# LuChengTHU/dpm-solver

Hardware: NVIDIA H100
Metric: solver-update GElem/s (higher is better)
Workload: dtype bf16

## Files before the change

dpm_solver_b200/_lib.py:

```python
from __future__ import annotations

import ctypes as C
import os
from pathlib import Path

_PKG = Path(__file__).resolve().parent
LIB_PATH = _PKG / "lib" / "libdpmsolver_b200.so"

DPM_F32, DPM_BF16, DPM_F16 = 0, 1, 2
FORM_NONE, FORM_LIN1, FORM_LIN2, FORM_LIN3, FORM_DIFF2, FORM_MS3, FORM_SS3T = range(7)
PARAM_NOISE, PARAM_X_START, PARAM_V, PARAM_SCORE = range(4)

PARAM_BY_NAME = {"noise": PARAM_NOISE, "x_start": PARAM_X_START, "v": PARAM_V, "score": PARAM_SCORE}


class StepDesc(C.Structure):
    _fields_ = [
        ("x", C.c_void_p), ("xe", C.c_void_p), ("m0", C.c_void_p), ("m1", C.c_void_p),
        ("m2", C.c_void_p), ("m_out", C.c_void_p), ("out", C.c_void_p), ("out2", C.c_void_p),
        ("e_cond", C.c_void_p), ("e_uncond", C.c_void_p), ("thr", C.c_void_p),
        ("n", C.c_uint64), ("per_sample", C.c_uint64),
        ("state_dtype", C.c_int32), ("model_dtype", C.c_int32), ("form", C.c_int32),
        ("n_model", C.c_int32), ("param", C.c_int32), ("predict_x0", C.c_int32),
        ("c0_on_old", C.c_int32), ("raw_round", C.c_int32),
# ... 41 lines not shown
    "dpm_dynamic_threshold_workspace": (C.c_size_t, [_u64, _u64]),
    "dpm_dynamic_threshold": (C.c_int, [_vp, C.POINTER(StepDesc), _f, _f, _vp, C.c_size_t, _vp]),
    "dpm_adaptive_init": (C.c_int, [C.POINTER(AdaptiveCtl), _f, _f, _vp]),
    "dpm_adaptive_plan": (C.c_int, [C.POINTER(AdaptiveCtl), _vp]),
    "dpm_adaptive_decide": (C.c_int, [C.POINTER(AdaptiveCtl), _vp]),
    "dpm_select_copy": (C.c_int, [_vp, _vp, _vp, _u64, _vp]),
    "dpm_adaptive_error_workspace": (C.c_size_t, [_u64, _u64]),
    "dpm_adaptive_error": (C.c_int, [_vp, _vp, _vp, _vp, _f, _f, _u64, _u64, _i, _vp, C.c_size_t, _vp]),
    "dpm_cfg_rescale_workspace": (C.c_size_t, [_u64, _u64]),
    "dpm_cfg_rescale_ratio": (C.c_int, [_vp, _vp, _vp, _f, _u64, _u64, _i, _vp, C.c_size_t, _vp]),
    "dpm_step_rescaled": (C.c_int, [C.POINTER(StepDesc), _vp, _f, _f, _vp]),
    "dpm_step_guided": (C.c_int, [C.POINTER(StepDesc), _vp, _vp, _f, _f, _vp]),
    "dpm_cfg_rescale_ratio_guided": (C.c_int, [_vp, _vp, _vp, _vp, _u64, _u64, _i, _vp, C.c_size_t, _vp]),
    "dpm_step_multi": (C.c_int, [C.POINTER(StepDesc), C.POINTER(_vp), C.POINTER(_f), _i, C.POINTER(_vp), _vp]),
    "dpm_replicate": (C.c_int, [_vp, _vp, _u64, _i, _i, _vp]),
}

MAX_CONDITIONS = 4

_lib = None


class DpmLibraryError(RuntimeError):
    pass


def lib() -> C.CDLL:
    global _lib
    if _lib is not None:
        return _lib
# ... 22 lines not shown
```

dpm_solver_b200/build.py:

```python
from __future__ import annotations

import argparse
import hashlib
import os
import shutil
import subprocess
import sys
from concurrent.futures import ThreadPoolExecutor
from pathlib import Path

PKG = Path(__file__).resolve().parent
ROOT = PKG.parent
CSRC = PKG / "csrc"
INCLUDE = ROOT / "include"
OUT_DIR = PKG / "lib"
BUILD_DIR = PKG / "build"
LIB_NAME = "libdpmsolver_b200.so"

SOURCES = ["capi.cu", "step_direct.cu", "step_multi.cu", "step_tma.cu","quantile.cu", "adaptive.cu", "adaptive_ctl.cu", "philox.cu"]
FMAD_DEFAULT = {"philox.cu"}
ARCH = ["-gencode", "arch=compute_90a,code=sm_90a"]
NVCC_FLAGS = ["-O3", "-std=c++17", "-lineinfo", "-fmad=false", "-Xcompiler", "-fPIC",
              "-Xcompiler", "-fvisibility=hidden", "--expt-relaxed-constexpr"]


def _nvcc() -> str:
    for cand in (os.environ.get("NVCC"), shutil.which("nvcc"), "/usr/local/cuda/bin/nvcc"):
        if cand and Path(cand).exists():
            return cand
    raise RuntimeError("nvcc not found (set NVCC=/path/to/nvcc)")


def _stamp(extra: list[str]) -> str:
    h = hashlib.sha256()
# ... 62 lines not shown
```

dpm_solver_b200/csrc/capi.cu:

```cuda
#include <atomic>
#include <mutex>
#include <set>
#include <utility>
#include <cstdarg>
#include <cstdio>
#include <cstdlib>
#include <cstring>

#include "launch.cuh"

namespace dpm {

static thread_local char g_err[512] = "";
static std::atomic<uint64_t> g_launches{0};
static std::atomic<int> g_variant{2}, g_threads{0}, g_ctas{0};

void set_error(const char* fmt, ...) {
  va_list ap;
  va_start(ap, fmt);
  vsnprintf(g_err, sizeof(g_err), fmt, ap);
  va_end(ap);
}
void count_launch() { g_launches.fetch_add(1, std::memory_order_relaxed); }
bool pdl_enabled() {
// ... 260 lines not shown
  Tuning t{g_variant.load(), g_threads.load(), g_ctas.load()};
  bool body_done = false;
  if (mp.k.npk > 0 && aligned_all && mp.k.dev_coef == nullptr) {
    const int r = launch_step_multi(mp, t, stream);
    if (r < 0 || r > 1) return r;
    body_done = (r == 0);
  }
  if (!body_done) {
    rc = launch_step_multi_scalar(mp, stream);
  } else if (mp.k.n % kPacket) {
    rc = launch_step_multi_scalar(shifted_multi(mp, (uint64_t)mp.k.npk * kPacket), stream);
  }
  return finish(rc);
}

}

using namespace dpm;

extern "C" {

int dpm_version(void) { return DPM_B200_VERSION; }
const char* dpm_last_error(void) { return g_err; }
uint64_t dpm_launch_count(void) { return g_launches.load(); }

int dpm_set_tuning(int variant, int threads, int ctas_per_sm) {
  if (variant < 0 || variant > 2) { set_error("variant must be 0 (direct), 1 (TMA ring) or 2 (auto)"); return DPM_ERR_ARG; }
  if (threads != 0 && (threads < 32 || threads > 512 || threads % 32)) { set_error("threads must be a multiple of 32 in [32,512]"); return DPM_ERR_ARG; }
  if (ctas_per_sm < 0 || ctas_per_sm > 32) { set_error("ctas_per_sm must be in [0,32]"); return DPM_ERR_ARG; }
  g_variant = variant; g_threads = threads; g_ctas = ctas_per_sm;
// ... 135 lines not shown
  if (out == nullptr || x == nullptr || !valid_dtype(dtype)) { set_error("duplicate: NULL tensor or bad dtype"); return DPM_ERR_ARG; }
  cudaStream_t st = static_cast<cudaStream_t>(stream);
  const uint64_t bytes = n * (uint64_t)esize(dtype);
  int r = launch_duplicate(out, x, bytes, st);
  if (r == 1) {
    cudaError_t e = cudaMemcpyAsync(out, x, bytes, cudaMemcpyDeviceToDevice, st);
    if (e == cudaSuccess) e = cudaMemcpyAsync(static_cast<char*>(out) + bytes, x, bytes, cudaMemcpyDeviceToDevice, st);
    return e != cudaSuccess ? launch_error("duplicate", e) : DPM_OK;
  }
  return finish(r);
}

int dpm_step_multi(const dpm_step_desc* desc, const void* const* e_conds, const float* scales, int n_cond,
                   void* const* replicas, dpm_stream_t stream) {
  return step_multi_impl(desc, e_conds, scales, n_cond, replicas, static_cast<cudaStream_t>(stream));
}

int dpm_replicate(void* out, const void* x, uint64_t n, int copies, int dtype, dpm_stream_t stream) {
  if (copies < 1 || out == nullptr || x == nullptr || !valid_dtype(dtype)) {
    set_error("replicate: NULL tensor, bad dtype or copies < 1");
    return DPM_ERR_ARG;
  }
  if (n == 0) return DPM_OK;
  cudaStream_t st = static_cast<cudaStream_t>(stream);
  const uint64_t bytes = n * (uint64_t)esize(dtype);
  int r = launch_replicate(out, x, bytes, copies, st);
  if (r == 1) {
    cudaError_t e = cudaSuccess;
    for (int c = 0; c < copies && e == cudaSuccess; ++c)
      e = cudaMemcpyAsync(static_cast<char*>(out) + (uint64_t)c * bytes, x, bytes, cudaMemcpyDeviceToDevice, st);
// ... 75 lines not shown
```

dpm_solver_b200/csrc/common.cuh:

```cuda
#pragma once
#include <cuda_bf16.h>
#include <cuda_fp16.h>
#include <cuda_runtime.h>
#include <stdint.h>
#include <string.h>

#include "dpm_solver_b200.h"

namespace dpm {

constexpr int kPacket = 8;

struct KParams {
  const void* x;
  const void* xe;
  const void* m0;
  const void* m1;
  const void* m2;
  const void* ec;
  const void* eu;
  void* m_out;
  void* out;
  void* out2;
  const float* thr;
// ... 21 lines not shown
  const float* dev_coef;
  const float* ratio;
  float phi, psi;
  const float* gscale;
};

constexpr int kMaxCond = DPM_MAX_CONDITIONS;
struct MultiParams {
  KParams k;
  const void* ec[kMaxCond];
  void* rep[kMaxCond];
  float s[kMaxCond];
  int32_t n_cond;
};

template <typename T> struct Raw;
template <> struct Raw<float> { uint32_t r[8]; };
template <> struct Raw<__nv_bfloat16> { uint32_t r[4]; };
template <> struct Raw<__half> { uint32_t r[4]; };

template <typename T> struct Traits;
template <> struct Traits<float> { static constexpr int kBytes = 4; static constexpr int kCode = DPM_F32; };
template <> struct Traits<__nv_bfloat16> { static constexpr int kBytes = 2; static constexpr int kCode = DPM_BF16; };
template <> struct Traits<__half> { static constexpr int kBytes = 2; static constexpr int kCode = DPM_F16; };

__device__ __forceinline__ void ldg_pk(Raw<float>& v, const float* p) {
  asm volatile("ld.global.L1::no_allocate.v4.b32 {%0,%1,%2,%3}, [%8];\n\t"
               "ld.global.L1::no_allocate.v4.b32 {%4,%5,%6,%7}, [%8+16];"
               : "=r"(v.r[0]), "=r"(v.r[1]), "=r"(v.r[2]), "=r"(v.r[3]), "=r"(v.r[4]),
                 "=r"(v.r[5]), "=r"(v.r[6]), "=r"(v.r[7])
// ... 357 lines not shown
```

dpm_solver_b200/csrc/launch.cuh:

```cuda
#pragma once
#include <cuda_runtime.h>
#include <stdint.h>

#include <type_traits>

#include "common.cuh"

namespace dpm {

struct Tuning {
  int variant;
  int threads;
  int ctas_per_sm;
};

int sm_count();
int max_smem_optin();
void count_launch();
int ensure_max_smem(const void* kernel, bool nonportable_cluster = false);
void set_error(const char* fmt, ...);
int launch_error(const char* what, cudaError_t e);

template <typename TE_, typename TS_> struct PacketPair {
  using TE = TE_;
// ... 64 lines not shown
int launch_step_direct(const KParams& p, const Tuning& t, cudaStream_t stream);
int launch_step_scalar(const KParams& p, cudaStream_t stream);
int launch_step_tma(const KParams& p, const Tuning& t, cudaStream_t stream);
void philox_policy(uint64_t numel, uint32_t* grid, uint64_t* counter_offset);
int launch_noise_philox(void* out, const void* x, const void* xt, const float* mask, uint64_t mask_n, uint64_t n,
                        int t_count, const float* alpha, const float* sigma, uint64_t seed, uint64_t offset,
                        int x_dtype, int out_dtype, cudaStream_t stream);
int launch_adaptive_init(const dpm_adaptive_ctl* a, float t_T, float h_init, cudaStream_t stream);
int launch_adaptive_plan(const dpm_adaptive_ctl* a, cudaStream_t stream);
int launch_adaptive_decide(const dpm_adaptive_ctl* a, cudaStream_t stream);
int launch_select_copy(void* dst, const void* src, const float* state, uint64_t bytes, cudaStream_t stream);
int launch_duplicate(void* dst, const void* src, uint64_t bytes, cudaStream_t stream);
int launch_step_multi(const MultiParams& mp, const Tuning& t, cudaStream_t stream);
int launch_step_multi_scalar(const MultiParams& mp, cudaStream_t stream);
int launch_replicate(void* dst, const void* src, uint64_t bytes, int copies, cudaStream_t stream);
int launch_quantile(float* s_out, const KParams& p, uint64_t n_samples, float q, float max_val,
                    void* workspace, size_t workspace_bytes, cudaStream_t stream);
size_t quantile_workspace_bytes(uint64_t n_samples, uint64_t per_sample);
size_t adaptive_workspace_bytes(uint64_t n, uint64_t per_sample);
int launch_adaptive_error(float* out, const void* xh, const void* xl, const void* xp, float atol, float rtol,
                          uint64_t per_sample, uint64_t n, int dtype, void* ws, size_t ws_bytes, cudaStream_t stream);
size_t cfg_rescale_workspace_bytes(uint64_t n_samples, uint64_t per_sample);
int launch_cfg_rescale_ratio(float* ratio, const void* ec, const void* eu, float guidance, uint64_t per_sample,
                             uint64_t n, int dtype, void* ws, size_t ws_bytes, cudaStream_t stream,
                             const float* gscale = nullptr);

}
```

dpm_solver_b200/ops.py:

```python
from __future__ import annotations

import ctypes as C
from dataclasses import dataclass
from typing import Optional, Tuple

import torch

from . import _lib
from ._lib import (DPM_BF16, DPM_F16, DPM_F32, FORM_DIFF2, FORM_LIN1, FORM_LIN2, FORM_LIN3,
                   FORM_MS3, FORM_NONE, FORM_SS3T, PARAM_NOISE, StepDesc)

_DTYPE_CODE = {torch.float32: DPM_F32, torch.bfloat16: DPM_BF16, torch.float16: DPM_F16}
SUPPORTED_DTYPES = tuple(_DTYPE_CODE)


@dataclass
class StepArgs:
    form: int = FORM_NONE
    n_model: int = 0
    x: Optional[torch.Tensor] = None
    xe: Optional[torch.Tensor] = None
    m0: Optional[torch.Tensor] = None
    m1: Optional[torch.Tensor] = None
    m2: Optional[torch.Tensor] = None
# ... 17 lines not shown
    w3: float = 0.0
    w4: float = 0.0
    want_m_out: bool = False
    state_dtype: Optional[torch.dtype] = None
    out: Optional[torch.Tensor] = None
    out2: Optional[torch.Tensor] = None
    m_out: Optional[torch.Tensor] = None
    raw_round: int = 0
    coef_dev: Optional[torch.Tensor] = None
    ratio: Optional[torch.Tensor] = None
    phi: float = 0.0
    guidance_b: Optional[torch.Tensor] = None
    e_conds: Optional[Tuple[torch.Tensor, ...]] = None
    scales: Optional[Tuple[float, ...]] = None
    replicas: Optional[Tuple[torch.Tensor, ...]] = None

    def state_tensors(self):
        return [t for t in (self.x, self.xe, self.m0, self.m1, self.m2) if t is not None]

    def model_tensors(self):
        return [t for t in (self.e_cond, self.e_uncond) if t is not None]

    def reference_tensor(self) -> torch.Tensor:
        for t in (self.x, self.xe, self.e_cond, self.m0):
            if t is not None:
                return t
        raise ValueError("StepArgs without tensors")


_raw_stream = getattr(torch._C, "_cuda_getCurrentRawStream", None)
if _raw_stream is None:
    def _raw_stream(idx):
        return torch.cuda.current_stream(idx).cuda_stream


class CudaBackend:

    name = "cuda-sm90a"

    def __init__(self):
        self._lib = _lib.lib()

# ... 76 lines not shown
        if a.coef_dev is not None:
            cd = a.coef_dev
            if not cd.is_cuda or cd.dtype != torch.float32 or cd.numel() < 16 or not cd.is_contiguous() or cd.device != dev:
                raise TypeError("dpm_solver_b200: `coef_dev` must be 16 contiguous fp32 values on the tensors' device")
            keep.append(cd)
            d.dev_coef = cd.data_ptr()
        return d, keep, ref, sdt, layout

    def _new_like(self, ref, sdt, layout):
        if layout == "cl":
            return torch.empty(ref.shape, dtype=sdt, device=ref.device,
                               memory_format=torch.channels_last if ref.dim() == 4 else torch.channels_last_3d)
        return torch.empty(ref.shape, dtype=sdt, device=ref.device)

    def step(self, a: StepArgs) -> Tuple[Optional[torch.Tensor], Optional[torch.Tensor]]:
        d, keep, ref, sdt, layout = self._fill(a)
        m_out = out = None
        if a.n_model > 0 and (a.want_m_out or a.form == FORM_NONE):
            m_out = a.m_out if a.m_out is not None else self._new_like(ref, sdt, layout)
            self._check(m_out, "m_out", ref.device, ref.numel(), sdt)
            if self._layout(m_out) != layout:
                raise ValueError("dpm_solver_b200: preallocated m_out must be dense and laid out like the inputs")
            d.m_out = m_out.data_ptr()
        if a.form != FORM_NONE:
            out = a.out if a.out is not None else self._new_like(ref, sdt, layout)
            self._check(out, "out", ref.device, ref.numel(), sdt)
            if self._layout(out) != layout:
                raise ValueError("dpm_solver_b200: preallocated out must be dense and laid out like the inputs")
            d.out = out.data_ptr()
            if a.out2 is not None:
                self._check(a.out2, "out2", ref.device, ref.numel(), sdt)
                if self._layout(a.out2) != layout:
                    raise ValueError("dpm_solver_b200: out2 must be dense and laid out like out")
                d.out2 = a.out2.data_ptr()
        for v, what in ((a.ratio, "ratio"), (a.guidance_b, "guidance_b")):
            if v is None:
                continue
            if not v.is_cuda or v.dtype != torch.float32 or not v.is_contiguous() or v.device != ref.device:
                raise TypeError(f"dpm_solver_b200: `{what}` must be a contiguous fp32 tensor on the tensors' device")
            if a.per_sample <= 0 or ref.numel() % a.per_sample or v.numel() != ref.numel() // a.per_sample:
                raise ValueError(f"dpm_solver_b200: `{what}` needs one value per sample")
        if a.e_conds is not None:
            self._step_multi(a, d, ref, sdt, layout, keep)
        elif a.guidance_b is not None:
            self._launch(ref.device, self._lib.dpm_step_guided, C.byref(d), C.c_void_p(a.guidance_b.data_ptr()),
                         C.c_void_p(None if a.ratio is None else a.ratio.data_ptr()), C.c_float(a.phi),
                         C.c_float(1.0 - a.phi))
        elif a.ratio is not None:
            self._launch(ref.device, self._lib.dpm_step_rescaled, C.byref(d), C.c_void_p(a.ratio.data_ptr()),
                         C.c_float(a.phi), C.c_float(1.0 - a.phi))
        else:
            self._launch(ref.device, self._lib.dpm_step, C.byref(d))
        return m_out, out

    def _step_multi(self, a: StepArgs, d, ref, sdt, layout, keep) -> None:
        K = len(a.e_conds)
        if not 2 <= K <= _lib.MAX_CONDITIONS or a.scales is None or len(a.scales) != K or a.n_model != 2:
            raise ValueError("dpm_solver_b200: a multi-condition step takes 2..{} conditional outputs, one scale each, "
                             "and n_model == 2".format(_lib.MAX_CONDITIONS))
        if a.replicas is not None and len(a.replicas) != K:
            raise ValueError("dpm_solver_b200: a multi-condition step takes one replica per condition")
        n, mdt = ref.numel(), a.e_cond.dtype
        ecs = [self._check(e, "e_conds[%d]" % k, ref.device, n, mdt, layout) for k, e in enumerate(a.e_conds)]
        keep.extend(ecs)
        reps = None
        if a.replicas is not None and a.form != FORM_NONE:
            for k, r in enumerate(a.replicas):
                self._check(r, "replicas[%d]" % k, ref.device, n, sdt)
# ... 150 lines not shown
        with torch.cuda.device(x.device):
            seed, offset = self._philox_state(x.device, n, self._lib, generator)
        self._launch(x.device, self._lib.dpm_diffedit_corrector, C.c_void_p(out.data_ptr()), C.c_void_p(x.data_ptr()),
                     C.c_void_p(x0.data_ptr()), C.c_void_p(mask.data_ptr()), C.c_uint64(mask.numel()), C.c_uint64(n),
                     C.c_float(alpha), C.c_float(sigma), C.c_uint64(seed), C.c_uint64(offset), C.c_int(_DTYPE_CODE[x.dtype]))
        return out

    def prepare(self, a: StepArgs) -> Optional["PreparedStep"]:
        return PreparedStep.build(self, a)

    def launch_count(self) -> int:
        return int(self._lib.dpm_launch_count())

    def set_tuning(self, variant: int = 2, threads: int = 0, ctas_per_sm: int = 0) -> None:
        _lib.check(self._lib.dpm_set_tuning(variant, threads, ctas_per_sm))


class AdaptiveController:

    SUPPORTED = ("discrete", "linear")

    def __init__(self, be: "CudaBackend", ns, device, order: int, predict_x0: bool, taylor: bool, t_0: float,
                 theta: float, t_err: float, discrete_input: bool):
        if ns.schedule not in self.SUPPORTED:
            raise ValueError("the device controller supports the 'discrete' and 'linear' schedules")
        self.be, self.dev = be, torch.device(device)
        f32 = dict(dtype=torch.float32, device=self.dev)
        self.state = torch.zeros(16, **f32)
        self.coef = torch.zeros(4, 16, **f32)
        self.times = torch.zeros(6, **f32)
# ... 45 lines not shown
        st = self.state.cpu().view(torch.int32)
        return int(st[6]), int(st[5]), int(st[8])


class PreparedStep:

    __slots__ = ("be", "d", "ref_d", "fn", "n", "dev", "dev_index", "sdt", "mdt", "shape", "shape2", "need_out",
                 "need_m", "fields", "dup", "ptrs", "esize")

    ORDER = ("x", "xe", "m0", "m1", "m2", "e_cond", "e_uncond")
    _PTR = {"x": 0, "xe": 1, "m0": 2, "m1": 3, "m2": 4, "m_out": 5, "out": 6, "out2": 7, "e_cond": 8, "e_uncond": 9}

    @staticmethod
    def build(be: "CudaBackend", a: StepArgs) -> Optional["PreparedStep"]:
        if a.thr is not None or a.raw_round or a.ratio is not None or a.guidance_b is not None \
                or a.e_conds is not None or a.out is not None and a.out2 is None:
            return None
        ref = a.reference_tensor()
        if not ref.is_contiguous():
            return None
        for t in a.state_tensors() + a.model_tensors():
            if not t.is_contiguous() or t.device != ref.device:
                return None
        d, keep, ref, sdt, layout = be._fill(a)
        if layout != "c":
            return None
        self = PreparedStep()
        self.be, self.d, self.ref_d, self.fn = be, d, C.byref(d), be._lib.dpm_step
        self.n, self.dev, self.dev_index = ref.numel(), ref.device, ref.device.index
        self.sdt = sdt
        self.mdt = a.e_cond.dtype if a.e_cond is not None else sdt
# ... 79 lines not shown
```

dpm_solver_b200/solver.py:

```python
from __future__ import annotations

import dataclasses
import inspect
import math
from dataclasses import dataclass
from typing import List, Optional

import torch
import torch.distributed as dist

from . import ops, plan as P
from ._lib import FORM_LIN1, FORM_NONE, FORM_SS3T, PARAM_BY_NAME, PARAM_NOISE
from .ops import StepArgs

__all__ = ["model_wrapper", "DPM_Solver", "WrappedModel"]

_DEV = object()



@dataclass
class RawOutput:
    e_cond: torch.Tensor
    e_uncond: Optional[torch.Tensor]
# ... 465 lines not shown
        return self._RR_CODE.get(raw.e_cond.dtype, 0)

    @staticmethod
    def _rr_coeffs(co: P.Coeffs, code: int) -> P.Coeffs:
        if co.form != FORM_SS3T or not co.r_tensor:
            return co
        T = torch.bfloat16 if code == 1 else torch.float16
        rT = lambda v: float(torch.tensor(v, dtype=torch.float32).to(T))
        r1t, r2t = bool(co.r_tensor & 1), bool(co.r_tensor & 2)
        return dataclasses.replace(co, w0=rT(co.w0) if r1t else co.w0, w1=rT(co.w1) if r2t else co.w1,
                                   w2=rT(co.w2) if r2t else co.w2, w3=rT(co.w3) if r1t else co.w3,
                                   w4=co.w4)

    def _post_model(self, raw: RawOutput, xe, t_dev, alsig, co: Optional[P.Coeffs] = None, x=None,
                    m1=None, m2=None, want_m: bool = True, dup_out: bool = False, x0: Optional[bool] = None,
                    slot=None):
        be = ops.backend()
        pkey = None
        if slot is not None and self._prep_on:
            pkey = (slot, raw.param, raw.guidance, raw.phi, raw.guidance_b is None, raw.e_uncond is None,
                    raw.e_cond.dtype, xe.dtype, xe.shape, want_m, dup_out, raw.scales)
            prep = self._prep_cache.get(pkey)
            if prep is not None:
                r = prep.launch((x, xe, raw.e_cond, m1, m2, raw.e_cond, raw.e_uncond))
                if r is not None:
                    m_new, x_next, x_in = r
                    if x_in is not None:
                        self._xin_pair = (x_next, x_in)
                    if m_new is None and prep.d.n_model == 0:
                        m_new = raw.e_cond
                    return m_new, x_next
# ... 48 lines not shown
            if q_raw is not None:
                qa = self._conv_args(q_raw, xe, alsig, sd, x0)
                qa.per_sample, qa.coef_dev = a.per_sample, a.coef_dev
            a.thr = be.dynamic_threshold(qa, float(self.dynamic_thresholding_ratio),
                                         float(self.thresholding_max_val))
        if custom_fix or co is None:
            a.form = FORM_NONE
            a.raw_round = rr & 3
            m_new = be.step(a)[0]
            if custom_fix:
                m_new = self._state_like(self.correcting_x0_fn(m_new, t_dev), sd)
            x_next = self._pure_update(co, x, m_new, m1, m2, rr=rr & 4 and rr) if co is not None else None
            return m_new, x_next
        self._fill_update(a, co, x, m1, m2)
        a.want_m_out = want_m
        a.raw_round = rr
        dup = self._dup_target(x) if dup_out else None
        if dup is not None:
            if a.e_conds is not None:
                a.out, a.replicas = dup[1], dup[2:]
            else:
                a.out, a.out2 = dup[1], dup[2]
        m_new, x_next = be.step(a)
        if dup is not None:
            self._xin_pair = (x_next, dup[0])
        if pkey is not None and not a.per_sample and a.e_conds is None:
            self._remember(pkey, a, dup)
        return m_new, x_next

    def _remember(self, pkey, a: StepArgs, dup=None) -> None:
        if dup is not None:
            a.out, a.out2 = dup[1], dup[2]
        prep = ops.backend().prepare(a)
        if prep is not None:
            if len(self._prep_cache) >= 512:
                self._prep_cache.clear()
            self._prep_cache[pkey] = prep

    @staticmethod
    def _state_like(t, sd):
        if t.dtype != sd:
            t = t.to(sd)
        return t if ops.CudaBackend._layout(t) is not None else t.contiguous()

    @staticmethod
    def _fill_update(a: StepArgs, co: P.Coeffs, x, m1, m2) -> None:
        a.form, a.x, a.m1, a.m2 = co.form, x, m1, m2
        if co.dev is not None:
            a.coef_dev = co.dev
        a.a, a.c0, a.c1, a.c2 = co.a, co.c0, co.c1, co.c2
        a.w0, a.w1, a.w2, a.w3, a.w4 = co.w0, co.w1, co.w2, co.w3, co.w4
        a.c0_on_old = co.c0_on_old

    def _pure_update(self, co: P.Coeffs, x, m0, m1=None, m2=None, rr: Optional[int] = None, pkey=None):
        if rr is None:
# ... 375 lines not shown
                key = ("multistep", steps, order, skip_type, t_T, t_0, solver_type, lower_order_final)

                def build():
                    ts = self.get_time_steps(skip_type=skip_type, t_T=t_T, t_0=t_0, N=steps, device='cpu')
                    assert ts.shape[0] - 1 == steps
                    marg = P.Marginals(ns, ts)
                    plan = P.multistep_plan(ns, self.algorithm_type, solver_type, ts, order, lower_order_final,
                                            marginals=marg)
                    return ts, plan, list(zip(marg.alpha.tolist(), marg.sigma.tolist()))

                ts, plan, alsig = self._host_plan(key, build)
                plan = self._sync_plan(plan, key)
                _, _, ts_dev, _, tin = self._device_tables(key, ts, x.shape[0], device)
                step = 0
                pid = self._plan_id(key)
                raw = self._evaluate(x, ts_dev[0], None if tin is None else tin[0])
                xe = x
                if self.correcting_xt_fn is not None:
                    x = self._state_like(self.correcting_xt_fn(x, ts_dev[0], step), sd)
                if return_intermediate:
                    intermediates.append(x)
                older: List[torch.Tensor] = []
                for step in range(1, steps + 1):
                    co = plan[step - 1]
                    m1 = older[-1] if co.order >= 2 else None
                    m2 = older[-2] if co.order >= 3 else None
                    want = order >= 2 and step < steps
                    m_new, x_new = self._post_model(raw, xe, ts_dev[step - 1], alsig[step - 1], co, x,
                                                    m1, m2, want_m=want, dup_out=step < steps,
                                                    slot=(pid, step))
                    x = x_new
                    t = ts_dev[step]
                    if self.correcting_xt_fn is not None:
                        x = self._state_like(self.correcting_xt_fn(x, t, step), sd)
                    if return_intermediate:
                        intermediates.append(x)
                    if m_new is not None:
                        older.append(m_new)
                        if len(older) > 2:
                            older.pop(0)
                    if step < steps:
                        raw = self._evaluate(x, t, None if tin is None else tin[step])
                        xe = x
            elif method in ['singlestep', 'singlestep_fixed']:
                key = (method, steps, order, skip_type, t_T, t_0, solver_type)
# ... 70 lines not shown
```

include/dpm_solver_b200.h:

```cpp
#ifndef DPM_SOLVER_B200_H
#define DPM_SOLVER_B200_H

#include <stddef.h>
#include <stdint.h>

#ifdef __cplusplus
extern "C" {
#endif

#define DPM_B200_VERSION 102

#if defined(__GNUC__)
#define DPM_API __attribute__((visibility("default")))
#else
#define DPM_API
#endif

typedef void* dpm_stream_t;

typedef enum dpm_status {
  DPM_OK = 0,
  DPM_ERR_ARG = -1,
  DPM_ERR_UNSUPPORTED = -2,
  DPM_ERR_ALIGN = -3
} dpm_status;
// ... 118 lines not shown
                                  void* workspace, size_t workspace_bytes, dpm_stream_t stream);
DPM_API int dpm_step_rescaled(const dpm_step_desc* desc, const float* ratio, float phi, float one_minus_phi,
                              dpm_stream_t stream);

DPM_API int dpm_step_guided(const dpm_step_desc* desc, const float* guidance, const float* ratio, float phi,
                            float one_minus_phi, dpm_stream_t stream);
DPM_API int dpm_cfg_rescale_ratio_guided(float* ratio_out, const void* e_cond, const void* e_uncond,
                                         const float* guidance, uint64_t per_sample, uint64_t n, int model_dtype,
                                         void* workspace, size_t workspace_bytes, dpm_stream_t stream);

#define DPM_MAX_CONDITIONS 4
DPM_API int dpm_step_multi(const dpm_step_desc* desc, const void* const* e_conds, const float* scales, int n_cond,
                           void* const* replicas, dpm_stream_t stream);
DPM_API int dpm_replicate(void* out, const void* x, uint64_t n, int copies, int dtype, dpm_stream_t stream);

typedef struct dpm_adaptive_ctl {
  int32_t schedule_kind;
  int32_t table_len;
  const float* t_array;
  const float* log_alpha_array;
  const float* log_alpha_flipped;
  const float* t_flipped;
  float beta_0, beta_1_minus_beta_0, inv_total_N;
  int32_t discrete_time_input;
  int32_t order;
  int32_t predict_x0;
  int32_t taylor;
  float t_0, theta, t_err;
  float* state;
  float* coef;
// ... 15 lines not shown
```

Before: 306.2.

## Store multistep history buffers in a lossless compressed packed bf16 format

Adds a packed encoding for the model-output history (m1/m2). Each group of 8 bf16 values is stored as sign plus low mantissa bytes, 4-bit exponent offsets and a per-packet base exponent, with a raw fallback when the exponents span too wide a range. A new step kernel reads and writes these packed buffers, so the memory-bound solver update moves fewer bytes per history tensor. The cost is extra encode/decode integer work, scattered byte loads and stores, a fallback path that touches more memory, and prepared-step caching being turned off when packing is enabled.

```diff
diff --git a/dpm_solver_b200/_lib.py b/dpm_solver_b200/_lib.py
--- a/dpm_solver_b200/_lib.py
+++ b/dpm_solver_b200/_lib.py
@@ -79,6 +79,9 @@
     "dpm_cfg_rescale_ratio_guided": (C.c_int, [_vp, _vp, _vp, _vp, _u64, _u64, _i, _vp, C.c_size_t, _vp]),
     "dpm_step_multi": (C.c_int, [C.POINTER(StepDesc), C.POINTER(_vp), C.POINTER(_f), _i, C.POINTER(_vp), _vp]),
     "dpm_replicate": (C.c_int, [_vp, _vp, _u64, _i, _i, _vp]),
+    "dpm_packed_bytes": (C.c_size_t, [_u64]),
+    "dpm_step_packed": (C.c_int, [C.POINTER(StepDesc), _vp, _vp, _vp, _vp]),
+    "dpm_unpack": (C.c_int, [_vp, _vp, _u64, _vp]),
 }
 
 MAX_CONDITIONS = 4
diff --git a/dpm_solver_b200/build.py b/dpm_solver_b200/build.py
--- a/dpm_solver_b200/build.py
+++ b/dpm_solver_b200/build.py
@@ -17,7 +17,7 @@
 BUILD_DIR = PKG / "build"
 LIB_NAME = "libdpmsolver_b200.so"
 
-SOURCES = ["capi.cu", "step_direct.cu", "step_multi.cu", "step_tma.cu","quantile.cu", "adaptive.cu", "adaptive_ctl.cu", "philox.cu"]
+SOURCES = ["capi.cu", "step_direct.cu", "step_multi.cu", "step_packed.cu", "step_tma.cu","quantile.cu", "adaptive.cu", "adaptive_ctl.cu", "philox.cu"]
 FMAD_DEFAULT = {"philox.cu"}
 ARCH = ["-gencode", "arch=compute_90a,code=sm_90a"]
 NVCC_FLAGS = ["-O3", "-std=c++17", "-lineinfo", "-fmad=false", "-Xcompiler", "-fPIC",
diff --git a/dpm_solver_b200/csrc/capi.cu b/dpm_solver_b200/csrc/capi.cu
--- a/dpm_solver_b200/csrc/capi.cu
+++ b/dpm_solver_b200/csrc/capi.cu
@@ -298,6 +298,39 @@
   return finish(rc);
 }
 
+static inline bool aligned16(const void* p) { return (reinterpret_cast<uintptr_t>(p) & 15) == 0; }
+
+static int step_packed_impl(const dpm_step_desc* desc, const void* m1, const void* m2, void* m_out,
+                            cudaStream_t stream) {
+  if (desc != nullptr && desc->n == 0) return DPM_OK;
+  if (desc == nullptr || desc->state_dtype != DPM_BF16 || desc->model_dtype != DPM_BF16 || desc->n % kPacket ||
+      desc->raw_round != 0 || desc->dev_coef != nullptr) {
+    set_error("packed step: needs a bf16 state and network output, n %% 8 == 0, raw_round == 0 and no dev_coef");
+    return DPM_ERR_ARG;
+  }
+  dpm_step_desc d = *desc;
+  d.m0 = nullptr; d.m1 = m1; d.m2 = m2; d.m_out = nullptr;
+  PackedParams pp;
+  memset(&pp, 0, sizeof(pp));
+  Needs nd;
+  int rc = build_params(&d, &pp.k, &nd, false);
+  if (rc != DPM_OK) return rc;
+  if (!packed_served(pp.k) || !fast_path_ok(pp.k)) {
+    set_error("packed step: form %d / n_model %d / this parameterisation has no packed kernel", d.form, d.n_model);
+    return DPM_ERR_ARG;
+  }
+  if (!all_aligned(pp.k, nd) || (m_out != nullptr && !aligned16(m_out))) {
+    set_error("packed step: every pointer must be 16-byte aligned");
+    return DPM_ERR_ARG;
+  }
+  pp.m1.p = nd.m1 ? static_cast<const uint8_t*>(m1) : nullptr;
+  pp.m2.p = nd.m2 ? static_cast<const uint8_t*>(m2) : nullptr;
+  pp.k.m1 = pp.k.m2 = nullptr;
+  pp.m_out.p = static_cast<uint8_t*>(m_out);
+  Tuning t{0, g_threads.load(), g_ctas.load()};
+  return finish(launch_step_packed(pp, t, stream));
+}
+
 }
 
 using namespace dpm;
@@ -463,6 +496,23 @@
 int dpm_step_multi(const dpm_step_desc* desc, const void* const* e_conds, const float* scales, int n_cond,
                    void* const* replicas, dpm_stream_t stream) {
   return step_multi_impl(desc, e_conds, scales, n_cond, replicas, static_cast<cudaStream_t>(stream));
+}
+
+int dpm_step_packed(const dpm_step_desc* desc, const void* m1_packed, const void* m2_packed, void* m_out_packed,
+                    dpm_stream_t stream) {
+  return step_packed_impl(desc, m1_packed, m2_packed, m_out_packed, static_cast<cudaStream_t>(stream));
+}
+
+size_t dpm_packed_bytes(uint64_t n) { return n % kPacket ? 0 : (size_t)packed_bytes(n / kPacket); }
+
+int dpm_unpack(const void* packed, void* out, uint64_t n, dpm_stream_t stream) {
+  if (n == 0) return DPM_OK;
+  if (packed == nullptr || out == nullptr || n % kPacket || (n >> 3) > 0xffffffffull || !aligned16(packed) ||
+      !aligned16(out)) {
+    set_error("unpack: needs non-NULL 16-byte aligned buffers and n %% 8 == 0 (at most 2^35-1 elements)");
+    return DPM_ERR_ARG;
+  }
+  return finish(launch_unpack(packed, out, (uint32_t)(n / kPacket), static_cast<cudaStream_t>(stream)));
 }
 
 int dpm_replicate(void* out, const void* x, uint64_t n, int copies, int dtype, dpm_stream_t stream) {
diff --git a/dpm_solver_b200/csrc/common.cuh b/dpm_solver_b200/csrc/common.cuh
--- a/dpm_solver_b200/csrc/common.cuh
+++ b/dpm_solver_b200/csrc/common.cuh
@@ -59,6 +59,88 @@
   int32_t n_cond;
 };
 
+constexpr uint64_t kPkGroup = 512;
+struct PackedRef {
+  const uint8_t* p;
+};
+struct PackedOut {
+  uint8_t* p;
+};
+struct PackedOffsets {
+  uint64_t r, s, e, b;
+};
+__host__ __device__ __forceinline__ uint64_t packed_bytes(uint64_t npk) { return 29 * npk; }
+__host__ __device__ __forceinline__ PackedOffsets packed_offsets(uint64_t npk, uint64_t pk) {
+  const uint64_t g0 = pk & ~(kPkGroup - 1), j = pk - g0;
+  const uint64_t gn = npk - g0 < kPkGroup ? npk - g0 : kPkGroup;
+  const uint64_t base = 16 * npk + 13 * g0;
+  return {16 * pk, base + 8 * j, base + 8 * gn + 4 * j, base + 12 * gn + j};
+}
+
+struct PackedParams {
+  KParams k;
+  PackedRef m1, m2;
+  PackedOut m_out;
+};
+
+#ifdef __CUDACC__
+__device__ __forceinline__ uint32_t prmt(uint32_t a, uint32_t b, uint32_t sel) {
+  uint32_t d;
+  asm("prmt.b32 %0, %1, %2, %3;" : "=r"(d) : "r"(a), "r"(b), "r"(sel));
+  return d;
+}
+__device__ __forceinline__ uint32_t max_u16x2(uint32_t a, uint32_t b) {
+  uint32_t d;
+  asm("max.u16x2 %0, %1, %2;" : "=r"(d) : "r"(a), "r"(b));
+  return d;
+}
+__device__ __forceinline__ uint32_t min_u16x2(uint32_t a, uint32_t b) {
+  uint32_t d;
+  asm("min.u16x2 %0, %1, %2;" : "=r"(d) : "r"(a), "r"(b));
+  return d;
+}
+__device__ __forceinline__ uint32_t lane_mask16(uint32_t v) { return prmt(v, 0u, 0xBB99u); }
+
+__device__ __forceinline__ void pk_encode(const uint32_t (&w)[4], uint2& s, uint32_t& e, uint32_t& base) {
+  uint32_t z[4], nz[4];
+#pragma unroll
+  for (int i = 0; i < 4; ++i) {
+    z[i] = w[i] & 0x7fff7fffu;
+    nz[i] = lane_mask16(z[i] + 0x7fff7fffu);
+  }
+  const uint32_t mx2 = max_u16x2(max_u16x2(z[0], z[1]), max_u16x2(z[2], z[3]));
+  const uint32_t mn2 = min_u16x2(min_u16x2(z[0] | ~nz[0], z[1] | ~nz[1]), min_u16x2(z[2] | ~nz[2], z[3] | ~nz[3]));
+  const uint32_t zmax = max(mx2 & 0xffffu, mx2 >> 16), zmin = min(mn2 & 0xffffu, mn2 >> 16);
+  const uint32_t emax = zmax >> 7, emin = zmin >> 7;
+  const bool esc = emax == 255u || zmin < 0x80u || emin + 14u < emax;
+  const uint32_t k2 = ((15u - emax) & 15u) * 0x00010001u;
+  uint32_t c[4];
+#pragma unroll
+  for (int i = 0; i < 4; ++i) c[i] = ((z[i] >> 7) + k2) & nz[i] & 0x000f000fu;
+  const uint32_t lo = c[0] + (c[1] << 8), hi = c[2] + (c[3] << 8);
+  e = esc ? 0u : lo + (hi << 4);
+  base = esc ? 0u : (emax == 0u ? 1u : emax);
+  const uint32_t lb0 = prmt(w[0], w[1], 0x6420u), hb0 = prmt(w[0], w[1], 0x7531u);
+  const uint32_t lb1 = prmt(w[2], w[3], 0x6420u), hb1 = prmt(w[2], w[3], 0x7531u);
+  s.x = (hb0 & 0x80808080u) | (lb0 & 0x7f7f7f7fu);
+  s.y = (hb1 & 0x80808080u) | (lb1 & 0x7f7f7f7fu);
+}
+
+__device__ __forceinline__ void pk_decode(uint2 s, uint32_t e, uint32_t base, uint32_t (&w)[4]) {
+  const uint32_t c7[4] = {(e << 7) & 0x07800780u, (e >> 1) & 0x07800780u, (e << 3) & 0x07800780u,
+                          (e >> 5) & 0x07800780u};
+  const uint32_t kb = (((base + 241u) & 0xffu) << 7) * 0x00010001u;
+  const uint32_t sw[4] = {s.x, s.x, s.y, s.y};
+#pragma unroll
+  for (int i = 0; i < 4; ++i) {
+    const uint32_t nz = lane_mask16(c7[i] + 0x7fff7fffu);
+    const uint32_t ex = (c7[i] + kb) & nz & 0x7f807f80u;
+    const uint32_t sb = prmt(sw[i], 0u, (i & 1) ? 0x3322u : 0x1100u);
+    w[i] = (sb & 0x807f807fu) | ex;
+  }
+}
+#endif
+
 template <typename T> struct Raw;
 template <> struct Raw<float> { uint32_t r[8]; };
 template <> struct Raw<__nv_bfloat16> { uint32_t r[4]; };
diff --git a/dpm_solver_b200/csrc/launch.cuh b/dpm_solver_b200/csrc/launch.cuh
--- a/dpm_solver_b200/csrc/launch.cuh
+++ b/dpm_solver_b200/csrc/launch.cuh
@@ -102,6 +102,9 @@
 int launch_step_multi(const MultiParams& mp, const Tuning& t, cudaStream_t stream);
 int launch_step_multi_scalar(const MultiParams& mp, cudaStream_t stream);
 int launch_replicate(void* dst, const void* src, uint64_t bytes, int copies, cudaStream_t stream);
+bool packed_served(const KParams& p);
+int launch_step_packed(const PackedParams& pp, const Tuning& t, cudaStream_t stream);
+int launch_unpack(const void* packed, void* out, uint32_t npk, cudaStream_t stream);
 int launch_quantile(float* s_out, const KParams& p, uint64_t n_samples, float q, float max_val,
                     void* workspace, size_t workspace_bytes, cudaStream_t stream);
 size_t quantile_workspace_bytes(uint64_t n_samples, uint64_t per_sample);
diff --git a/dpm_solver_b200/csrc/step_packed.cu b/dpm_solver_b200/csrc/step_packed.cu
--- /dev/null
+++ b/dpm_solver_b200/csrc/step_packed.cu
@@ -0,0 +1,189 @@
+#include "common.cuh"
+#include "launch.cuh"
+
+namespace dpm {
+
+constexpr int kPkUnroll = 2;
+
+__device__ __forceinline__ uint2 ldg_s(const uint2* p) {
+  uint2 v;
+  asm volatile("ld.global.L1::no_allocate.v2.b32 {%0,%1}, [%2];" : "=r"(v.x), "=r"(v.y) : "l"(p));
+  return v;
+}
+__device__ __forceinline__ uint32_t ldg_e(const uint32_t* p) {
+  uint32_t v;
+  asm volatile("ld.global.L1::no_allocate.b32 %0, [%1];" : "=r"(v) : "l"(p));
+  return v;
+}
+__device__ __forceinline__ uint32_t ldg_b(const uint8_t* p) {
+  uint16_t v;
+  asm volatile("ld.global.L1::no_allocate.u8 %0, [%1];" : "=h"(v) : "l"(p));
+  return v;
+}
+__device__ __forceinline__ void stg_s(uint2* p, uint2 v) {
+  asm volatile("st.global.L1::no_allocate.v2.b32 [%0], {%1,%2};" ::"l"(p), "r"(v.x), "r"(v.y) : "memory");
+}
+__device__ __forceinline__ void stg_e(uint32_t* p, uint32_t v) {
+  asm volatile("st.global.L1::no_allocate.b32 [%0], %1;" ::"l"(p), "r"(v) : "memory");
+}
+__device__ __forceinline__ void stg_b(uint8_t* p, uint32_t v) {
+  asm volatile("st.global.L1::no_allocate.u8 [%0], %1;" ::"l"(p), "h"((uint16_t)v) : "memory");
+}
+
+__device__ __forceinline__ void pk_load(Raw<__nv_bfloat16>& v, const PackedRef& src, const PackedOffsets& o, uint2 s,
+                                        uint32_t e, uint32_t b) {
+  if (b != 0u) {
+    pk_decode(s, e, b, v.r);
+  } else {
+    ldg_pk(v, reinterpret_cast<const __nv_bfloat16*>(src.p + o.r));
+  }
+}
+__device__ __forceinline__ void pk_fetch(const PackedRef& src, const PackedOffsets& o, uint2& s, uint32_t& e,
+                                         uint32_t& b) {
+  s = ldg_s(reinterpret_cast<const uint2*>(src.p + o.s));
+  e = ldg_e(reinterpret_cast<const uint32_t*>(src.p + o.e));
+  b = ldg_b(src.p + o.b);
+}
+__device__ __forceinline__ void pk_store(const PackedOut& dst, const PackedOffsets& o, const Raw<__nv_bfloat16>& v) {
+  uint2 s;
+  uint32_t e, b;
+  pk_encode(v.r, s, e, b);
+  stg_s(reinterpret_cast<uint2*>(dst.p + o.s), s);
+  stg_e(reinterpret_cast<uint32_t*>(dst.p + o.e), e);
+  stg_b(dst.p + o.b, b);
+  if (b == 0u) stg_pk(reinterpret_cast<__nv_bfloat16*>(dst.p + o.r), v);
+}
+
+template <int NE, int FORM>
+__global__ void __launch_bounds__(512) k_step_packed(const __grid_constant__ PackedParams pp) {
+  using T = __nv_bfloat16;
+  constexpr bool kM1 = form_reads(FORM).m1, kM2 = form_reads(FORM).m2;
+  const KParams& p = pp.k;
+  const T* __restrict__ gx = static_cast<const T*>(p.x);
+  const T* __restrict__ gxe = static_cast<const T*>(p.xe);
+  const T* __restrict__ gec = static_cast<const T*>(p.ec);
+  const T* __restrict__ geu = static_cast<const T*>(p.eu);
+  T* __restrict__ go = static_cast<T*>(p.out);
+  T* __restrict__ go2 = static_cast<T*>(p.out2);
+
+  const uint32_t npk = p.npk;
+  const uint32_t tile_pk = blockDim.x * kPkUnroll;
+  const bool sep_xe = p.use_xe && !p.xe_is_x;
+  const bool clamp = p.thr != nullptr;
+  pdl_trigger();
+  pdl_wait();
+
+  for (uint64_t tile0 = (uint64_t)blockIdx.x * tile_pk; tile0 < npk; tile0 += (uint64_t)gridDim.x * tile_pk) {
+    Raw<T> rx[kPkUnroll], rxe[kPkUnroll], rec[kPkUnroll], reu[kPkUnroll];
+    uint2 s1[kPkUnroll], s2[kPkUnroll];
+    uint32_t e1[kPkUnroll], e2[kPkUnroll], b1[kPkUnroll], b2[kPkUnroll];
+#pragma unroll
+    for (int u = 0; u < kPkUnroll; ++u) {
+      const uint64_t pk = tile0 + (uint64_t)u * blockDim.x + threadIdx.x;
+      if (pk < npk) {
+        const size_t e = (size_t)pk * kPacket;
+        ldg_pk(rx[u], gx + e);
+        ldg_pk(rec[u], gec + e);
+        if (NE == 2) ldg_pk(reu[u], geu + e);
+        if (sep_xe) ldg_pk(rxe[u], gxe + e);
+        if (kM1 || kM2) {
+          const PackedOffsets o = packed_offsets(npk, pk);
+          if (kM1) pk_fetch(pp.m1, o, s1[u], e1[u], b1[u]);
+          if (kM2) pk_fetch(pp.m2, o, s2[u], e2[u], b2[u]);
+        }
+      }
+    }
+#pragma unroll
+    for (int u = 0; u < kPkUnroll; ++u) {
+      const uint64_t pk = tile0 + (uint64_t)u * blockDim.x + threadIdx.x;
+      if (pk < npk) {
+        const size_t e = (size_t)pk * kPacket;
+        const PackedOffsets o = packed_offsets(npk, pk);
+        float fx[8], fxe[8], fT[8], fm1[8], fm2[8], fo[8], fec[8], feu[8];
+        unpack(rx[u], fx);
+        if (kM1) {
+          Raw<T> r;
+          pk_load(r, pp.m1, o, s1[u], e1[u], b1[u]);
+          unpack(r, fm1);
+        }
+        if (kM2) {
+          Raw<T> r;
+          pk_load(r, pp.m2, o, s2[u], e2[u], b2[u]);
+          unpack(r, fm2);
+        }
+        unpack(rec[u], fec);
+        if (NE == 2) unpack(reu[u], feu);
+        const float s_thr = clamp ? __ldg(p.thr + (uint32_t)pk / p.pk_per_sample) : 1.f;
+        if (sep_xe) {
+          unpack(rxe[u], fxe);
+          fast_model8<NE>(p, fxe, fec, feu, clamp, s_thr, fT);
+        } else {
+          fast_model8<NE>(p, fx, fec, feu, clamp, s_thr, fT);
+        }
+        Raw<T> rmo;
+        round_pack(rmo, fT);
+        if (pp.m_out.p != nullptr) pk_store(pp.m_out, o, rmo);
+        fast_update8<FORM>(p, fx, fT, fm1, fm2, fo);
+        Raw<T> ro;
+        pack(ro, fo);
+        stg_pk(go + e, ro);
+        if (go2 != nullptr) stg_pk(go2 + e, ro);
+      }
+    }
+  }
+}
+
+__global__ void __launch_bounds__(256) k_unpack(const PackedRef src, __nv_bfloat16* __restrict__ dst, uint32_t npk) {
+  for (uint64_t pk = (uint64_t)blockIdx.x * blockDim.x + threadIdx.x; pk < npk; pk += (uint64_t)gridDim.x * blockDim.x) {
+    const PackedOffsets o = packed_offsets(npk, pk);
+    Raw<__nv_bfloat16> v;
+    uint2 s;
+    uint32_t e, b;
+    pk_fetch(src, o, s, e, b);
+    pk_load(v, src, o, s, e, b);
+    stg_pk(dst + pk * kPacket, v);
+  }
+}
+
+typedef void (*PackedKernel)(const PackedParams);
+
+static PackedKernel pick_packed(const KParams& p) {
+  return with_form(p.form, [&](auto form) -> PackedKernel {
+    constexpr int FORM = decltype(form)::value;
+    if constexpr (FORM == DPM_FORM_LIN1 || FORM == DPM_FORM_LIN2 || FORM == DPM_FORM_DIFF2 || FORM == DPM_FORM_MS3) {
+      if (p.n_model == 1) return k_step_packed<1, FORM>;
+      if (p.n_model == 2) return k_step_packed<2, FORM>;
+    }
+    return nullptr;
+  });
+}
+
+bool packed_served(const KParams& p) { return pick_packed(p) != nullptr; }
+
+int launch_step_packed(const PackedParams& pp, const Tuning& t, cudaStream_t stream) {
+  PackedKernel k = pick_packed(pp.k);
+  if (k == nullptr) return 1;
+  const int threads = t.threads > 0 ? t.threads : 256;
+  const uint32_t tile_pk = (uint32_t)threads * kPkUnroll;
+  const uint64_t tiles = ((uint64_t)pp.k.npk + tile_pk - 1) / tile_pk;
+  const uint64_t cap = t.ctas_per_sm > 0 ? (uint64_t)sm_count() * t.ctas_per_sm : tiles;
+  const uint32_t grid = (uint32_t)(tiles < cap ? tiles : cap);
+  if (grid == 0) return 0;
+  cudaError_t le = launch_pdl(k, grid, (unsigned)threads, 0, stream, pp);
+  if (le != cudaSuccess) return launch_error("packed step launch failed", le);
+  count_launch();
+  return 0;
+}
+
+int launch_unpack(const void* packed, void* out, uint32_t npk, cudaStream_t stream) {
+  if (npk == 0) return 0;
+  const int threads = 256;
+  const uint64_t blocks = ((uint64_t)npk + threads - 1) / threads;
+  const uint64_t cap = (uint64_t)sm_count() * 16;
+  k_unpack<<<(uint32_t)(blocks < cap ? blocks : cap), threads, 0, stream>>>(PackedRef{static_cast<const uint8_t*>(packed)},
+                                                                          static_cast<__nv_bfloat16*>(out), npk);
+  count_launch();
+  return 0;
+}
+
+}
diff --git a/dpm_solver_b200/ops.py b/dpm_solver_b200/ops.py
--- a/dpm_solver_b200/ops.py
+++ b/dpm_solver_b200/ops.py
@@ -1,6 +1,8 @@
 from __future__ import annotations
 
 import ctypes as C
+import dataclasses
+import struct
 from dataclasses import dataclass
 from typing import Optional, Tuple
 
@@ -55,6 +57,7 @@
     e_conds: Optional[Tuple[torch.Tensor, ...]] = None
     scales: Optional[Tuple[float, ...]] = None
     replicas: Optional[Tuple[torch.Tensor, ...]] = None
+    pack_m_out: bool = False
 
     def state_tensors(self):
         return [t for t in (self.x, self.xe, self.m0, self.m1, self.m2) if t is not None]
@@ -67,6 +70,16 @@
             if t is not None:
                 return t
         raise ValueError("StepArgs without tensors")
+
+
+def _is_packed(t: Optional[torch.Tensor]) -> bool:
+    return t is not None and t.dtype == torch.uint8
+
+
+def _recip_div_ok(d: float) -> bool:
+    b = struct.unpack("<I", struct.pack("<f", d))[0]
+    ex = (b >> 23) & 0xff
+    return 107 <= ex <= 147 and (b & 0x7fffff) != 0x7fffff
 
 
 _raw_stream = getattr(torch._C, "_cuda_getCurrentRawStream", None)
@@ -173,6 +186,11 @@
         return torch.empty(ref.shape, dtype=sdt, device=ref.device)
 
     def step(self, a: StepArgs) -> Tuple[Optional[torch.Tensor], Optional[torch.Tensor]]:
+        if a.pack_m_out or _is_packed(a.m1) or _is_packed(a.m2):
+            r = self._step_packed(a)
+            if r is not None:
+                return r
+            a = dataclasses.replace(a, pack_m_out=False, m1=self._unpacked(a.m1, a), m2=self._unpacked(a.m2, a))
         d, keep, ref, sdt, layout = self._fill(a)
         m_out = out = None
         if a.n_model > 0 and (a.want_m_out or a.form == FORM_NONE):
@@ -182,16 +200,7 @@
                 raise ValueError("dpm_solver_b200: preallocated m_out must be dense and laid out like the inputs")
             d.m_out = m_out.data_ptr()
         if a.form != FORM_NONE:
-            out = a.out if a.out is not None else self._new_like(ref, sdt, layout)
-            self._check(out, "out", ref.device, ref.numel(), sdt)
-            if self._layout(out) != layout:
-                raise ValueError("dpm_solver_b200: preallocated out must be dense and laid out like the inputs")
-            d.out = out.data_ptr()
-            if a.out2 is not None:
-                self._check(a.out2, "out2", ref.device, ref.numel(), sdt)
-                if self._layout(a.out2) != layout:
-                    raise ValueError("dpm_solver_b200: out2 must be dense and laid out like out")
-                d.out2 = a.out2.data_ptr()
+            out = self._outputs(a, d, ref, sdt, layout)
         for v, what in ((a.ratio, "ratio"), (a.guidance_b, "guidance_b")):
             if v is None:
                 continue
@@ -211,6 +220,66 @@
         else:
             self._launch(ref.device, self._lib.dpm_step, C.byref(d))
         return m_out, out
+
+    def _outputs(self, a: StepArgs, d, ref, sdt, layout) -> torch.Tensor:
+        out = a.out if a.out is not None else self._new_like(ref, sdt, layout)
+        self._check(out, "out", ref.device, ref.numel(), sdt)
+        if self._layout(out) != layout:
+            raise ValueError("dpm_solver_b200: preallocated out must be dense and laid out like the inputs")
+        d.out = out.data_ptr()
+        if a.out2 is not None:
+            self._check(a.out2, "out2", ref.device, ref.numel(), sdt)
+            if self._layout(a.out2) != layout:
+                raise ValueError("dpm_solver_b200: out2 must be dense and laid out like out")
+            d.out2 = a.out2.data_ptr()
+        return out
+
+    _PACKED_FORMS = (FORM_LIN1, FORM_LIN2, FORM_DIFF2, FORM_MS3)
+
+    def packed_bytes(self, n: int) -> int:
+        return int(self._lib.dpm_packed_bytes(n))
+
+    def _step_packed(self, a: StepArgs):
+        bf = torch.bfloat16
+        if a.form not in self._PACKED_FORMS or a.n_model not in (1, 2) or a.param != PARAM_NOISE or a.raw_round \
+                or a.ratio is not None or a.guidance_b is not None or a.e_conds is not None or a.coef_dev is not None \
+                or a.m_out is not None or (a.want_m_out and not a.pack_m_out):
+            return None
+        if a.form != FORM_LIN1 and not _is_packed(a.m1) or a.form == FORM_MS3 and not _is_packed(a.m2):
+            return None
+        if a.state_dtype not in (None, bf) or any(t.dtype != bf for t in (a.x, a.xe, a.e_cond, a.e_uncond)
+                                                      if t is not None):
+            return None
+        n = a.x.numel()
+        if n % 8 or (a.thr is not None and a.per_sample % 8) or (a.predict_x0 and not _recip_div_ok(a.alpha_e)):
+            return None
+        d, keep, ref, sdt, layout = self._fill(dataclasses.replace(a, m1=None, m2=None))
+        nb = self.packed_bytes(n)
+        ms = [t if _is_packed(t) else None for t in (a.m1, a.m2)]
+        for t in ms:
+            if t is not None and (t.numel() != nb or t.device != ref.device or not t.is_contiguous()):
+                raise ValueError("dpm_solver_b200: a packed buffer holds dpm_packed_bytes(n) bytes on the tensors' device")
+        m_out = torch.empty(nb, dtype=torch.uint8, device=ref.device) if a.want_m_out else None
+        out = self._outputs(a, d, ref, sdt, layout)
+        ptrs = [d.x, d.xe, d.e_cond, d.e_uncond, d.out, d.out2] + [t.data_ptr() for t in ms + [m_out] if t is not None]
+        if any(p is not None and p % 16 for p in ptrs):
+            return None
+        self._launch(ref.device, self._lib.dpm_step_packed, C.byref(d), *[C.c_void_p(None if t is None else t.data_ptr())
+                                                                          for t in ms + [m_out]])
+        return m_out, out
+
+    def unpack(self, packed: torch.Tensor, like: torch.Tensor) -> torch.Tensor:
+        n = like.numel()
+        if packed.dtype != torch.uint8 or packed.numel() != self.packed_bytes(n) or not packed.is_contiguous() \
+                or packed.device != like.device:
+            raise ValueError("dpm_solver_b200: a packed buffer holds dpm_packed_bytes(n) bytes on the tensors' device")
+        out = self._new_like(like, torch.bfloat16, "cl" if self._layout(like) == "cl" else "c")
+        self._launch(like.device, self._lib.dpm_unpack, C.c_void_p(packed.data_ptr()), C.c_void_p(out.data_ptr()),
+                     C.c_uint64(n))
+        return out
+
+    def _unpacked(self, t: Optional[torch.Tensor], a: StepArgs) -> Optional[torch.Tensor]:
+        return self.unpack(t, a.reference_tensor()) if _is_packed(t) else t
 
     def _step_multi(self, a: StepArgs, d, ref, sdt, layout, keep) -> None:
         K = len(a.e_conds)
@@ -391,6 +460,11 @@
 
     def set_tuning(self, variant: int = 2, threads: int = 0, ctas_per_sm: int = 0) -> None:
         _lib.check(self._lib.dpm_set_tuning(variant, threads, ctas_per_sm))
+
+    def get_tuning(self) -> Tuple[int, int, int]:
+        v, t, c = C.c_int(), C.c_int(), C.c_int()
+        _lib.check(self._lib.dpm_get_tuning(C.byref(v), C.byref(t), C.byref(c)))
+        return v.value, t.value, c.value
 
 
 class AdaptiveController:
@@ -466,7 +540,8 @@
     @staticmethod
     def build(be: "CudaBackend", a: StepArgs) -> Optional["PreparedStep"]:
         if a.thr is not None or a.raw_round or a.ratio is not None or a.guidance_b is not None \
-                or a.e_conds is not None or a.out is not None and a.out2 is None:
+                or a.e_conds is not None or a.out is not None and a.out2 is None \
+                or a.pack_m_out or _is_packed(a.m1) or _is_packed(a.m2):
             return None
         ref = a.reference_tensor()
         if not ref.is_contiguous():
diff --git a/dpm_solver_b200/solver.py b/dpm_solver_b200/solver.py
--- a/dpm_solver_b200/solver.py
+++ b/dpm_solver_b200/solver.py
@@ -503,7 +503,7 @@
 
     def _post_model(self, raw: RawOutput, xe, t_dev, alsig, co: Optional[P.Coeffs] = None, x=None,
                     m1=None, m2=None, want_m: bool = True, dup_out: bool = False, x0: Optional[bool] = None,
-                    slot=None):
+                    slot=None, pack: bool = False):
         be = ops.backend()
         pkey = None
         if slot is not None and self._prep_on:
@@ -582,6 +582,7 @@
             return m_new, x_next
         self._fill_update(a, co, x, m1, m2)
         a.want_m_out = want_m
+        a.pack_m_out = pack and want_m
         a.raw_round = rr
         dup = self._dup_target(x) if dup_out else None
         if dup is not None:
@@ -605,8 +606,19 @@
                 self._prep_cache.clear()
             self._prep_cache[pkey] = prep
 
+    def _pack_buffers(self, x, order: int) -> bool:
+        be, w = ops.backend(), self._wrapped
+        if order < 2 or x.dtype != torch.bfloat16 or x.numel() % 8 or x.shape[0] <= 16 or self.reference_rounding:
+            return False
+        if not hasattr(be, "get_tuning") or be.get_tuning()[0] == 1:
+            return False
+        return not (isinstance(w, WrappedModel) and (w.guidance_rescale != 0 or w._scale_vec is not None
+                                                     or w.cond_scales is not None))
+
     @staticmethod
     def _state_like(t, sd):
+        if ops._is_packed(t):
+            return t
         if t.dtype != sd:
             t = t.to(sd)
         return t if ops.CudaBackend._layout(t) is not None else t.contiguous()
@@ -1012,6 +1024,9 @@
                 _, _, ts_dev, _, tin = self._device_tables(key, ts, x.shape[0], device)
                 step = 0
                 pid = self._plan_id(key)
+                pack = self._pack_buffers(x, order)
+                if pack:
+                    self._prep_on = False
                 raw = self._evaluate(x, ts_dev[0], None if tin is None else tin[0])
                 xe = x
                 if self.correcting_xt_fn is not None:
@@ -1026,7 +1041,7 @@
                     want = order >= 2 and step < steps
                     m_new, x_new = self._post_model(raw, xe, ts_dev[step - 1], alsig[step - 1], co, x,
                                                     m1, m2, want_m=want, dup_out=step < steps,
-                                                    slot=(pid, step))
+                                                    slot=(pid, step), pack=pack)
                     x = x_new
                     t = ts_dev[step]
                     if self.correcting_xt_fn is not None:
diff --git a/include/dpm_solver_b200.h b/include/dpm_solver_b200.h
--- a/include/dpm_solver_b200.h
+++ b/include/dpm_solver_b200.h
@@ -8,7 +8,7 @@
 extern "C" {
 #endif
 
-#define DPM_B200_VERSION 102
+#define DPM_B200_VERSION 103
 
 #if defined(__GNUC__)
 #define DPM_API __attribute__((visibility("default")))
@@ -157,6 +157,11 @@
                            void* const* replicas, dpm_stream_t stream);
 DPM_API int dpm_replicate(void* out, const void* x, uint64_t n, int copies, int dtype, dpm_stream_t stream);
 
+DPM_API size_t dpm_packed_bytes(uint64_t n);
+DPM_API int dpm_step_packed(const dpm_step_desc* desc, const void* m1_packed, const void* m2_packed, void* m_out_packed,
+                            dpm_stream_t stream);
+DPM_API int dpm_unpack(const void* packed, void* out, uint64_t n, dpm_stream_t stream);
+
 typedef struct dpm_adaptive_ctl {
   int32_t schedule_kind;
   int32_t table_len;
```

Result: faster. 318.9 (median of 6 runs) (+4.1%).
